# tatsy/normalizing-flows-pytorch

Hardware: AMD Instinct MI355X
Metric: samples/sec (train step: forward flow + log-det + NLL + backward + Adam) (higher is better)
Workload: dtype f32; 1 GPU; Glow CIFAR-shape (3,32,32) L=3 K=32 batch 64 per GPU (512 over 8); per_gpu_batch=64, global_batch=64, parallelism=dp1, hipgraph=True, deterministic=True, dp_one_graph=False

## Files before the change

include/nfhip.h:

```cpp
#ifndef NFHIP_H
#define NFHIP_H

#include <stdint.h>

#ifdef __cplusplus
extern "C" {
#endif

typedef void* nf_stream_t;

enum nf_split_mode {
    NF_SPLIT_1D = 0,
    NF_SPLIT_CHECKER = 1,
    NF_SPLIT_CHANNEL = 2,
    NF_SPLIT_NONE = 3
};

enum nf_chan_op {
    NF_ACTNORM = 0,
    NF_FLOWBN = 1
};

#define NF_E_BADARG 10001
#define NF_E_UNSUPPORTED 10002
// ... 332 lines not shown
    const float* cp_out;
    const float* cp_a;
    const float* cp_c;
    float* cp_g_z;
    float* cp_g_out;
    float* cp_g_a;
    float* cp_g_c;
    int cp_mode, cp_odd, cp_C;
    int ws_gen;
    float* g_gamma[5];
    float* g_beta[5];
    const float* wpk[6];
    const float* hd_g_h;
    const float* hd_W;
    const float* hd_ls;
} nf_convnet_bwd_desc;
int nf_convnet_chain_bwd(const nf_convnet_bwd_desc* desc, int64_t B, int I0, int O_out, int H, int W, int training,
                         nf_stream_t stream);
int nf_convnet_chain_bwd_run(const nf_convnet_bwd_desc* descs, int n, int64_t B, int I0, int O_out, int H, int W, int training,
                             nf_stream_t stream);

#define NF_CONV_PACK_IMAGE_FLOATS (3 * 36 * 128)
#define NF_CONV_PACK_MAX_LAYERS 1024
typedef struct nf_conv_pack_desc {
    const float* w;
    float* dst;
    int O, I, ksize, reserved;
} nf_conv_pack_desc;
int nf_conv_weight_pack_images(int O, int I, int ksize);
int nf_conv_weight_pack(const nf_conv_pack_desc* descs, int n, nf_stream_t stream);
// ... 450 lines not shown
```

normalizing-flows-pytorch_amd/csrc/conv_bn.hip:

```cpp
#include <mutex>
#include <unordered_set>
#include <vector>

#include "nf_common.h"
#include "nf_det.h"

NF_DET_STATE(nf_cvb)
NF_DET_HOST_API(nf_cvb)

#include "nf_conv_core.h"

#ifdef NF_CV_PROF
__device__ long long nf_cv_prof[32];
#define NF_CV_STAMP(i)                                                                 \
    do {                                                                               \
        if (blockIdx.x == 0 && threadIdx.x == 0) nf_cv_prof[i] = wall_clock64();       \
    } while (0)
extern "C" int nf_cv_prof_read(long long* out) {
    return (int)hipMemcpyFromSymbol(out, HIP_SYMBOL(nf_cv_prof), sizeof(long long) * 32);
}
#else
#define NF_CV_STAMP(i)
#endif

// ... 917 lines not shown
}
static_assert(sizeof(nf_conv_bwd_desc) % sizeof(unsigned) == 0, "descriptor: whole words");

static int nf_conv_bn_wgrad_launch(nf_conv_bwd_desc* descs, const nf_conv_bwd_desc* tab, int n, int slabs, int64_t B, int I, int O, int H,
                                   int W, int ksize, nf_stream_t stream) {
    NfCvGeo g;
    if (descs == nullptr || n < 1 || (tab == nullptr && n > NF_CV_WG_MAX) || n > NF_CONV_WGRAD_TABLE_MAX ||
        !nf_conv_bn_usable(B > 0 ? B : 1, I, O, H, W, ksize))
        return NF_E_BADARG;
    if (B == 0) return 0;
    if (!nf_cv_geometry(g, B, H, W, ksize)) return NF_E_BADARG;
    if (!nf_cv_fits_int32(B, I > O ? I : O, H * W)) return NF_E_BADARG;
    if (!nf_cv_set_valid(g, descs[0].valid_h, descs[0].valid_w)) return NF_E_BADARG;
    const bool masked = nf_cv_masked(g);
    bool one_plain = true;
    for (int k = 0; k < n; ++k) {
        if (descs[k].valid_h != descs[0].valid_h || descs[k].valid_w != descs[0].valid_w) return NF_E_BADARG;
        if (descs[k].g_weff == nullptr || descs[k].in == nullptr) return NF_E_BADARG;
        if (descs[k].bn_gamma != nullptr && I > 32) return NF_E_BADARG;
        if (descs[k].gn_src != nullptr && O > 32) return NF_E_BADARG;
        descs[k].g_store = nullptr; descs[k].gn_out = nullptr; descs[k].sum_g = nullptr; descs[k].sum_gx = nullptr;
        one_plain = one_plain && !(descs[k].g_direct != nullptr && descs[k].g_skip != nullptr);
    }
    NfCvBwdMulti m{};
    hipStream_t st = (hipStream_t)stream;
    if (tab == nullptr) {
        for (int k = 0; k < n; ++k) m.d[k] = descs[k];
    } else {
        for (int k0 = 0; k0 < n; k0 += NF_CV_DESC_WRITE) {
            const int cnt = n - k0 < NF_CV_DESC_WRITE ? n - k0 : NF_CV_DESC_WRITE;
            NfCvDescChunk w{};
            for (int k = 0; k < cnt; ++k) w.d[k] = descs[k0 + k];
            hipLaunchKernelGGL(k_conv_desc_write, dim3(1), dim3(256), 0, st, w, const_cast<nf_conv_bwd_desc*>(tab) + k0, cnt);
        }
        m = NfCvBwdMulti{};
    }
    const int ICB = (I + 31) / 32, OCB = (O + 31) / 32;
    const int T = ksize * ksize;
    const size_t lds = sizeof(float) * ((size_t)32 * g.CS + (size_t)32 * OCB * g.CS + 5 * 32 + 4 * 32 + 2 * 4 * 32);
    if (slabs < 1 || slabs > NF_CV_BWD_MAX_SLABS || slabs > g.tiles) return NF_E_BADARG;
    const unsigned grid = (unsigned)slabs;
    if (!masked && one_plain && nf_conv_bulk_wgrad_plan(B, I, O, H, W, ksize))
        return nf_conv_bulk_wgrad(tab == nullptr ? m.d : nullptr, tab, n, B, I, H, W, (int)grid, st);
    const int iters = (int)((g.tiles + grid - 1) / grid);
    int rc;
    const size_t lds_lean = sizeof(float) * ((size_t)2 * 64 * g.CS + 5 * 32 + 2 * 32);
    const bool lean = !masked && ICB == 1 && OCB == 1 && B * (int64_t)(I > O ? I : O) * H * W < ((int64_t)1 << 30) && 64 * g.CS >= T * 1024 &&
                      lds_lean <= 160 * 1024;
#define NF_LAUNCH(T_, IB_, OB_, LEAN_)                                                                                 \
    do {                                                                                                               \
        const size_t lds_ = LEAN_ ? lds_lean : lds;                                                                    \
        rc = nf_cv_optin(k_conv_bn_wgrad_multi<T_, IB_, OB_, LEAN_>, lds_);                                            \
        if (rc) return rc;                                                                                             \
        hipLaunchKernelGGL((k_conv_bn_wgrad_multi<T_, IB_, OB_, LEAN_>), dim3(grid, (unsigned)n), dim3(NF_CV_THREADS), lds_, st, m, \
                           tab, g, I, O, iters);                                                                       \
    } while (0)
    if (T == 9) {
        if (ICB == 1 && lean) NF_LAUNCH(9, 1, 1, true);
// ... 96 lines not shown
```

normalizing-flows-pytorch_amd/csrc/conv_bulk.hip:

```cpp
#include <cstdlib>
#include <mutex>
#include <type_traits>
#include <unordered_set>

#include "nf_common.h"
#include "nf_det.h"

NF_DET_STATE(nf_cbk)
NF_DET_HOST_API(nf_cbk)

#include "nf_conv_core.h"

#include "nf_bf16x3.h"

#ifdef NF_CB_PROF
__device__ long long nf_cb_prof[64];
#define NF_CB_STAMP(i)                                                                 \
    do {                                                                               \
        if (blockIdx.x == 0 && threadIdx.x == 0 && (i) < 64) nf_cb_prof[i] = wall_clock64(); \
    } while (0)
extern "C" int nf_cb_prof_read(long long* out) { return (int)hipMemcpyFromSymbol(out, HIP_SYMBOL(nf_cb_prof), sizeof(long long) * 64); }
#define NF_CBW_STAMP(T, i)                                                             \
    do {                                                                               \
        if (blockIdx.x == 0 && blockIdx.y == 0 && threadIdx.x == (T) && (i) >= 0 && (i) < 64) nf_cb_prof[i] = wall_clock64(); \
// ... 667 lines not shown
}
__device__ __forceinline__ const float* nf_cbw_pin(const float* p) {
    const uint64_t a = (uint64_t)p;
    const unsigned lo = __builtin_amdgcn_readfirstlane((unsigned)a), hi = __builtin_amdgcn_readfirstlane((unsigned)(a >> 32));
    return (const float*)(((uint64_t)hi << 32) | lo);
}
__device__ __forceinline__ void nf_cbw_put4(char* p, int plane_bytes, const float (&v)[4]) {
    bf16x2 h0, m0, l0, h1, m1, l1;
    nf_cc_split2(f32x2{v[0], v[1]}, h0, m0, l0);
    nf_cc_split2(f32x2{v[2], v[3]}, h1, m1, l1);
    *(bf16x4*)(p) = bf16x4{h0[0], h0[1], h1[0], h1[1]};
    *(bf16x4*)(p + plane_bytes) = bf16x4{m0[0], m0[1], m1[0], m1[1]};
    *(bf16x4*)(p + 2 * plane_bytes) = bf16x4{l0[0], l0[1], l1[0], l1[1]};
}

__global__ void __launch_bounds__(NF_CBW_THREADS) k_conv3_bulk_wgrad(NfCbwMulti m, const nf_conv_bwd_desc* __restrict__ tab, NfCbwGeo g, int I) {
    extern __shared__ __attribute__((aligned(16))) float smem[];
    const nf_conv_bwd_desc& d = tab != nullptr ? tab[blockIdx.y] : m.d[blockIdx.y];
    char* const lds = (char*)smem;
    const int PA = 32 * g.ACH, PG = 32 * NF_CBW_GCH;
    const int BUF = 3 * (PA + PG);
    float* cst = (float*)(lds + 2 * BUF);
    const int tid = threadIdx.x, lane = tid & 63, wid = __builtin_amdgcn_readfirstlane(tid >> 6), c32 = lane & 31, hs = lane >> 5;
    const bool walker = wid < 4;
    const bool has_bn = d.bn_gamma != nullptr, has_src = d.gn_src != nullptr;
    const int64_t Npx = g.B * g.HW;

    for (int e = tid; e < 2 * BUF / 16; e += NF_CBW_THREADS) *(u32x4*)(lds + 16 * e) = u32x4{0u, 0u, 0u, 0u};
    if (tid < 32) {
        const int oo = tid;
        float c1 = 0.f, mean = 0.f, invstd = 0.f, mg = 0.f, mgx = 0.f;
        if (has_src) {
            invstd = d.cbn_save_invstd[oo]; mean = d.cbn_save_mean[oo]; c1 = d.cbn_gamma[oo] * invstd;
            if (d.cbn_sum_g != nullptr) {
#pragma unroll
                for (int r = 0; r < NF_STAT_REPL; ++r) { mg += d.cbn_sum_g[32 * r + oo]; mgx += d.cbn_sum_gx[32 * r + oo]; }
                const float invN = 1.f / (float)Npx;
                mg *= invN; mgx *= invN;
            }
        }
// ... 135 lines not shown
                const bool ok = (cls == 1u || (cls == 2u && top) || (cls == 3u && bot)) && sm < brem;
                okm |= (ok ? 1u : 0u) << r;
                rx[S][r] = nf_cbw_ld128(rxs, ok ? xoff[r] : NF_CB_OOB);
            }
            xok[S] = okm;
            unsigned go[4], gp[4], gs[4];
#pragma unroll
            for (int r = 0; r < 4; ++r) {
                go[r] = pv ? goff0 + (unsigned)r * gcstep : NF_CB_OOB;
                gp[r] = plain != nullptr ? go[r] : NF_CB_OOB;
                gs[r] = has_src ? go[r] : NF_CB_OOB;
            }
            const __amdgpu_buffer_rsrc_t rr = nf_cb_rsrc(plain + gbase);
#pragma unroll
            for (int r = 0; r < 4; ++r) rp[S][r] = nf_cbw_ld128(rr, gp[r]);
            const __amdgpu_buffer_rsrc_t r3 = nf_cb_rsrc(p_src + gbase), r4 = nf_cb_rsrc(p_out + gbase);
#pragma unroll
            for (int r = 0; r < 4; ++r) { rs[S][r] = nf_cbw_ld128(r3, gs[r]); ro[S][r] = nf_cbw_ld128(r4, gs[r]); }
        };
        auto convert = [&](auto SET) {
            constexpr int S = decltype(SET)::value;
            char* fa = lds + S * BUF;
            char* fg = fa + 3 * PA;
#pragma unroll
            for (int r = 0; r < NF_CBW_MAXR; ++r)
                if (r < g.nr && ((xmeta >> (4 * r)) & 4u)) {
                    const bool ok = (xok[S] >> r) & 1u;
                    const float xsc = kx[r][0], xsh = kx[r][1];
                    float v[4];
#pragma unroll
                    for (int j = 0; j < 4; ++j) {
                        float x = rx[S][r][j];
                        if (has_bn) x = fmaxf(fmaf(x, xsc, xsh), 0.f);
                        v[j] = ok ? x : 0.f;
                    }
                    nf_cbw_put4(fa + xlds[r], PA, v);
                }
            float kg[4][5];
            if (has_src) {
#pragma unroll
                for (int r = 0; r < 4; ++r)
#pragma unroll
                    for (int q = 0; q < 5; ++q) kg[r][q] = cst[32 * q + 8 * r + gch0];
            }
#pragma unroll
            for (int r = 0; r < 4; ++r) {
                float v[4] = {0.f, 0.f, 0.f, 0.f};
                if (plain != nullptr) {
#pragma unroll
                    for (int j = 0; j < 4; ++j) v[j] = rp[S][r][j];
                }
                if (has_src) {
                    const float kc1 = kg[r][0], kmean = kg[r][1], kinv = kg[r][2], kmg = kg[r][3], kmgx = kg[r][4];
#pragma unroll
                    for (int j = 0; j < 4; ++j) {
                        const float xh = (ro[S][r][j] - kmean) * kinv;
                        v[j] += kc1 * (rs[S][r][j] - kmg - xh * kmgx);
                    }
                }
#pragma unroll
                for (int j = 0; j < 4; ++j) v[j] = gok[S] ? v[j] : 0.f;
                gsum[r] += (v[0] + v[1]) + (v[2] + v[3]);
                nf_cbw_put4(fg + glds0 + r * 8 * NF_CBW_GCH, PG, v);
            }
        };
        using S0 = std::integral_constant<int, 0>;
        using S1 = std::integral_constant<int, 1>;
        const int64_t n = tile0 < g.tiles ? (g.tiles - tile0 + tstep - 1) / tstep : 0;
        issue(S0{}, tile0);
        issue(S1{}, tile0 + tstep);
        if (n > 0) convert(S0{});
        issue(S0{}, tile0 + 2 * tstep);
// ... 394 lines not shown
#undef NF_CB_FWD2
#undef NF_CB_FWD3
    if (rc) return rc;
    NF_CHECK_LAUNCH();
    return 0;
}

extern "C" int nf_conv_bulk_wgrad_plan(int64_t B, int I, int O, int H, int W, int ksize) {
    const int on = 1;
    const int64_t min_px = nf_cb_min_px() == 16384 + 1 ? 4096 : nf_cb_min_px() - 1;
    if (!on || !nf_cb_on() || ksize != 3 || O != 32 || I < 1 || I > 32 || B * H * W < min_px) return 0;
    NfCbwGeo g;
    return nf_cbw_geometry(g, B, H, W) ? 1 : 0;
}
int nf_conv_bulk_wgrad(const nf_conv_bwd_desc* descs, const nf_conv_bwd_desc* tab, int n, int64_t B, int I, int H, int W, int slabs,
                       hipStream_t st) {
    NfCbwGeo g;
    if (!nf_cbw_geometry(g, B, H, W) || n < 1 || slabs < 1 || (descs == nullptr) == (tab == nullptr)) return NF_E_BADARG;
    if (descs != nullptr && n > NF_CONV_WGRAD_MAX) return NF_E_BADARG;
    NfCbwMulti m{};
    if (descs != nullptr)
        for (int k = 0; k < n; ++k) m.d[k] = descs[k];
    const size_t lds = nf_cbw_lds_bytes(g);
    int rc = nf_cb_optin(k_conv3_bulk_wgrad);
    if (rc) return rc;
    const unsigned gx = (unsigned)(g.tiles < slabs ? g.tiles : slabs);
    if ((int)gx != slabs) return NF_E_BADARG;
    hipLaunchKernelGGL(k_conv3_bulk_wgrad, dim3(gx, (unsigned)n), dim3(NF_CBW_THREADS), lds, st, m, tab, g, I);
    NF_CHECK_LAUNCH();
    return 0;
}

int nf_conv_bulk_bwd_plan(const nf_conv_bwd_desc* d, int64_t B, int I, int O, int H, int W, int ksize) {
    if (!nf_cb_on() || ksize != 3 || O != 32 || I < 1 || I > 32 || B * H * W < nf_cb_min_px()) return 0;
    if (d->g_weff != nullptr || d->g_bias != nullptr || d->g_direct != nullptr || d->gn_src == nullptr || d->out == nullptr) return 0;
    if (!(B * 32 * (int64_t)H * W < (int64_t)1 << 31)) return 0;
    NfCbGeo cg;
    return nf_cb_plan(cg, B, 32, H, W, 4, nf_cb_force_nblk());
}

int nf_conv_bulk_bwd(const nf_conv_bwd_desc* desc, int64_t B, int I, int H, int W, hipStream_t st) {
    NfCbGeo cg;
    const int nblk = nf_cb_plan(cg, B, 32, H, W, 4, nf_cb_force_nblk());
// ... 34 lines not shown
```

normalizing-flows-pytorch_amd/csrc/conv_chain.hip:

```cpp
#include <cstdlib>
#include <cstring>
#include <mutex>
#include <unordered_set>
#include "nf_conv_core.h"
#include "nf_det.h"

NF_DET_STATE(nf_ccd)
NF_DET_HOST_API(nf_ccd)
#include "nf_bf16x3.h"
#include "nf_small_plu.h"

#define NF_CC_NL 6
#define NF_CC_NB 5
#define NF_CC_MAX_BLOCKS NF_CONVNET_MAX_BLOCKS

#define NF_CC_WG_SLOTS (NF_CC_NB * NF_CC_MAX_BLOCKS * 64)
#define NF_CC_GROUP 16
#define NF_CC_MAX_GROUPS ((NF_CC_MAX_BLOCKS + NF_CC_GROUP - 1) / NF_CC_GROUP)
#define NF_CC_FLAT_MAX 128
#define NF_CC_STAT_SLOTS (NF_CC_WG_SLOTS + NF_CC_NB * NF_CC_MAX_GROUPS * 64)
static_assert(2 * NF_CC_STAT_SLOTS == NF_CONVNET_WS_FLOATS, "exchange workspace size in include/nfhip.h");

NF_PERSIST_STATE(nf_cc)
NF_PERSIST_HOST_API(nf_cc)
// ... 1544 lines not shown
        nrows = (G + NF_CC_GROUP - 1) / NF_CC_GROUP;
    }
    nf_cc_collect_slots<RUN>(xs, rs, gen, nrows, XS);
    peek();
    __syncthreads();
    {
        float pa = 0.f, pb = 0.f;
        for (int b = l; b < nrows; b += 32) { pa += xs[b * XS + ci]; pb += xs[b * XS + 32 + ci]; }
        const float A = nf_cc_sum32(pa), Bs = nf_cc_sum32(pb);
        if (l == 0) { tot[ci] = A; tot[32 + ci] = Bs; }
    }
    __syncthreads();
    return tot;
}

template <int NPB, int NKQ, bool HALO, bool CPL, int FWc, int CSc, bool PK, bool RUN>
__device__ __forceinline__ void nf_cc_bwd_step(const nf_convnet_bwd_desc& d, const NfCvGeo& g, int I0, int O_out, int training,
                                               const NfSplit& cs) {
    static_assert(NPB * NKQ == NF_CV_WAVES, "sixteen waves");
    constexpr int OWN = 16 / NKQ, PXW = 32 * NPB;
    extern __shared__ __attribute__((aligned(16))) float sm[];
    const NfCcLds L = nf_cc_lds<NPB, NKQ>(g.CS, 1);
    float* Wl = sm + L.WL;
    float* RS = sm + L.RS;
    float* kc = sm + L.KC;
    float* red = sm + L.RED;
    const int CSr = FWc > 0 ? CSc : g.CS;
    const int WPs = L.WPs;
    const int tid = nf_cc_step_tid<RUN>();
    const int lane = tid & 63, wid = tid >> 6, c32 = lane & 31, hs = lane >> 5;
// ... 205 lines not shown
                atomicAdd(d.cp_g_a, ta);
                atomicAdd(d.cp_g_c, tc);
            }
        }
        nf_cc_ksplit_exchange<NKQ>(own, acc, RS, pb, kq, lane);
        NF_CC_STAMP(67 + 6 * (4 - l));
        float* gn = d.gn[l];
#pragma unroll
        for (int rr = 0; rr < OWN; ++rr) {
            const int oc = nf_cv_cd_row(OWN * kq + rr, hs);
            const float a = xh[rr];
            const bool keep = pv && fmaf(a, kc[oc], kc[32 + oc]) > 0.f;
            const float v = keep ? own[rr] : 0.f;
            own[rr] = v;
            xh[rr] = (a - kc[64 + oc]) * kc[96 + oc];
            if (pv) gn[(b * 32 + oc) * g.HW + q] = v;
        }
        if (halo) nf_cc_halo_publish<OWN>(hslots, gbase, l, g, (int)tile, y0, px, kq, hs, own);
        float mg[OWN], mgx[OWN];
        unsigned long long hw[2] = {0ull, 0ull};
        const float* tot;
        {
            float p2[OWN], S1, S2;
            int which;
#pragma unroll
            for (int rr = 0; rr < OWN; ++rr) p2[rr] = own[rr] * xh[rr];
            nf_cc_half_sums2<OWN>(own, p2, c32, S1, S2, which);
            if (c32 < OWN) {
                const int oc = nf_cv_cd_row(OWN * kq + which, hs);
                red[pb * 32 + oc] = S1;
                red[NPB * 32 + pb * 32 + oc] = S2;
// ... 5 lines not shown
            if (stash) {
                if (blockIdx.x == 0 && nf_cc_tidx<RUN>() < 64) sm[ST + 64 * l + nf_cc_tidx<RUN>()] = tot[nf_cc_tidx<RUN>()];
            } else if (blockIdx.x == 0 && nf_cc_tidx<RUN>() < 64) {
                (nf_cc_tidx<RUN>() < 32 ? d.sum_g[l] : d.sum_gx[l])[nf_cc_tidx<RUN>() & 31] = tot[nf_cc_tidx<RUN>()];
                float* sink = nf_cc_tidx<RUN>() < 32 ? d.g_beta[l] : d.g_gamma[l];
                if (sink != nullptr) sink[nf_cc_tidx<RUN>() & 31] += tot[nf_cc_tidx<RUN>()];
            }
#pragma unroll
            for (int rr = 0; rr < OWN; ++rr) {
                const int oc = nf_cv_cd_row(OWN * kq + rr, hs);
                mg[rr] = training ? tot[oc] * invN : 0.f;
                mgx[rr] = training ? tot[32 + oc] * invN : 0.f;
            }
        }
        const bool on_stream = (l & 1) == 0;
        float* gs = (l == 4) ? d.g_store[0] : (l == 2 ? d.g_store[1] : nullptr);
#pragma unroll
        for (int rr = 0; rr < OWN; ++rr) {
            const int oc = nf_cv_cd_row(OWN * kq + rr, hs);
            float G = kc[oc] * (own[rr] - mg[rr] - xh[rr] * mgx[rr]);
            if (on_stream) G += gstream[rr];
            G = pv ? G : 0.f;
            own[rr] = G;
            if (on_stream) gstream[rr] = G;
            if (gs != nullptr && pv) gs[(b * 32 + oc) * g.HW + q] = G;
        }
#pragma unroll
        for (int j = 0; j < OWN / 4; ++j) {
            const int c0 = nf_cv_cd_row(OWN * kq + 4 * j, hs);
            nf_cc_frame_store4(Fr, CSr, c0, fpos, own[4 * j], own[4 * j + 1], own[4 * j + 2], own[4 * j + 3]);
        }
        if constexpr (OWN == 2) nf_cc_frame_store2(Fr, CSr, nf_cv_cd_row(OWN * kq, hs), fpos, own[0], own[1]);
        if constexpr (OWN == 1) nf_cc_frame_store1(Fr, CSr, nf_cv_cd_row(kq, hs), fpos, own[0]);
        if (halo && nf_cc_tidx<RUN>() < 32 * g.W) {
            const int c = nf_cc_tidx<RUN>() >> g.lgW;
            const float mgc = training ? tot[c] * invN : 0.f, mgxc = training ? tot[32 + c] * invN : 0.f;
#pragma unroll
            for (int s2 = 0; s2 < 2; ++s2) {
                float v = 0.f;
                const int f = nf_cc_halo_poll(hslots, gbase, l, g, (int)tile, y0, s2, v, hw[s2]);
// ... 390 lines not shown
    NF_CHECK_LAUNCH();
    return 0;
}

static int nf_cc_bwd_args(const nf_convnet_bwd_desc* desc, int64_t B, int I0, int O_out, int H, int W, NfSplit& cs, NfCvGeo& g, int& PX) {
    if (desc == nullptr || !nf_convnet_chain_usable(B, I0, O_out, H, W)) return NF_E_BADARG;
    memset(&cs, 0, sizeof(cs));
    if (desc->cp_g_y != nullptr) {
        if (desc->cp_g_ld == nullptr || desc->cp_z == nullptr || desc->cp_out == nullptr || desc->cp_a == nullptr || desc->cp_c == nullptr ||
            desc->cp_g_z == nullptr || desc->cp_g_out == nullptr || desc->cp_g_a == nullptr || desc->cp_g_c == nullptr)
            return NF_E_BADARG;
        if (!nf_cc_coupling_split(cs, desc->cp_mode, desc->cp_odd, desc->cp_C, I0, O_out, H, W)) return NF_E_BADARG;
    } else if (desc->g_out == nullptr) {
        return NF_E_BADARG;
    }
    PX = nf_cc_tile_px(B, H, W);
    if (!nf_cv_geometry(g, B, H, W, 3, PX)) return NF_E_BADARG;
    if (desc->hd_g_h != nullptr) {
        const bool small = desc->cp_C >= 2 && desc->cp_C <= 4;
        if (desc->cp_g_y == nullptr || desc->hd_W == nullptr || desc->hd_ls == nullptr || (!small && (desc->cp_C < 9 || desc->cp_C > 64)) ||
            ((cs.H * cs.W) & 15) != 0 || (H * W > PX && cs.W < 16) || (int64_t)(O_out >> 1) * PX > NF_CC_HD_X1_MAX)
            return NF_E_BADARG;
    }
    const bool pk = desc->wpk[0] != nullptr;
    for (int i = 1; i < NF_CC_NL; ++i)
        if ((desc->wpk[i] != nullptr) != pk) return NF_E_BADARG;
    return 0;
}

extern "C" int nf_convnet_chain_bwd(const nf_convnet_bwd_desc* desc, int64_t B, int I0, int O_out, int H, int W, int training,
// ... 122 lines not shown
```

normalizing-flows-pytorch_amd/csrc/nf_conv_core.h:

```cpp
#pragma once
#include "nf_common.h"

typedef float f32x16 __attribute__((ext_vector_type(16)));

#define NF_CV_WAVES 16
#define NF_CV_THREADS (NF_CV_WAVES * NF_WAVE)
#define NF_CV_PX 128
#define NF_CV_MAX_FRAME 384
#define NF_CV_FJ (NF_CV_MAX_FRAME / NF_WAVE)
#define NF_CV_CU (32 / NF_CV_WAVES)
#define NF_CV_MAX_I 96
#define NF_CV_MAX_O 192
#define NF_CV_WS 33
#define NF_CV_RS (NF_CV_WAVES * 12 * NF_WAVE)

struct NfCvGeo {
    int H, W, HW;
    int TH;
    int SEG;
    int halo;
    int FW, FS;
    int FSZ;
    int CS;
    int lgW, lgSP;
// ... 271 lines not shown
            sc = d.bn_gamma[k] * invstd;
            sh = d.bn_beta[k] - mean * sc;
        }
        kc[k] = sc;
        kc[32 + k] = sh;
    }
    if (training && d.bn_gamma != nullptr && d.bn_num_batches != nullptr && blockIdx.x == 0 && threadIdx.x == 0)
        d.bn_num_batches[0] += 1;
}

int nf_conv_bulk_fwd_plan(const nf_conv_desc* d, int64_t B, int I, int O, int H, int W, int ksize);
int nf_conv_bulk_fwd(const nf_conv_desc* desc, int64_t B, int I, int H, int W, int training, float eps, float mom, hipStream_t st);
int nf_conv_bulk_bwd_plan(const nf_conv_bwd_desc* d, int64_t B, int I, int O, int H, int W, int ksize);
int nf_conv_bulk_bwd(const nf_conv_bwd_desc* desc, int64_t B, int I, int H, int W, hipStream_t st);
extern "C" int nf_conv_bulk_wgrad_plan(int64_t B, int I, int O, int H, int W, int ksize);
int nf_conv_bulk_wgrad(const nf_conv_bwd_desc* descs, const nf_conv_bwd_desc* tab, int n, int64_t B, int I, int H, int W, int slabs, hipStream_t st);
int nf_conv1_bulk_fwd_plan(const nf_conv_desc* d, int64_t B, int I, int O, int H, int W, int ksize);
int nf_conv1_bulk_fwd(const nf_conv_desc* desc, int64_t B, int O, int H, int W, int training, float eps, float mom, hipStream_t st);
int nf_conv1_bulk_bwd_plan(const nf_conv_bwd_desc* d, int64_t B, int I, int O, int H, int W, int ksize);
int nf_conv1_bulk_bwd(const nf_conv_bwd_desc* desc, int64_t B, int O, int H, int W, hipStream_t st);
```

normalizing-flows-pytorch_amd/fused_conv.py:

```python
import ctypes
import functools

import torch

from . import _native as N
from . import workspace as WS
from .fused import BN_EPS, BN_MOMENTUM, H, R, _desc

WS_ROWS = 2 * R + 2
GB = 256

_FWD_FIELDS = ['in_', 'weight', 'bias', 'residual', 'out', 'bn_gamma', 'bn_beta', 'bn_sum', 'bn_sqsum', 'bn_center',
               'bn_running_mean', 'bn_running_var', 'bn_num_batches', 'bn_save_mean', 'bn_save_invstd', 'stat_sum',
               'stat_sqsum', 'wpk']
_BWD_FIELDS = ['in_', 'weight', 'bn_gamma', 'bn_beta', 'bn_save_mean', 'bn_save_invstd', 'g_direct', 'g_skip', 'gn_src',
               'out', 'cbn_gamma', 'cbn_save_mean', 'cbn_save_invstd', 'cbn_sum_g', 'cbn_sum_gx', 'g_store', 'g_bias',
               'g_weff', 'gn_out', 'sum_g', 'sum_gx', 'wpk']


class ConvDesc(ctypes.Structure):
    _fields_ = [(f, ctypes.c_void_p) for f in _FWD_FIELDS] + [('valid_h', ctypes.c_int), ('valid_w', ctypes.c_int)]


class ConvBwdDesc(ctypes.Structure):
# ... 18 lines not shown
                ('hs_P', ctypes.c_void_p), ('hs_L', ctypes.c_void_p), ('hs_U', ctypes.c_void_p), ('hs_Lm', ctypes.c_void_p),
                ('hs_Um', ctypes.c_void_p), ('hs_sign', ctypes.c_void_p), ('hs_Wout', ctypes.c_void_p),
                ('ws_gen', ctypes.c_int), ('ws_reserved', ctypes.c_int)]


class ConvNetBwdDesc(ctypes.Structure):
    _fields_ = [('w', ctypes.c_void_p * 6), ('gamma', ctypes.c_void_p * 5), ('beta', ctypes.c_void_p * 5),
                ('save_mean', ctypes.c_void_p * 5), ('save_invstd', ctypes.c_void_p * 5), ('acts', ctypes.c_void_p * 5),
                ('g_out', ctypes.c_void_p), ('gn', ctypes.c_void_p * 5), ('sum_g', ctypes.c_void_p * 5),
                ('sum_gx', ctypes.c_void_p * 5), ('g_store', ctypes.c_void_p * 2), ('g_x', ctypes.c_void_p),
                ('ws_zero', ctypes.c_void_p),
                ('cp_g_y', ctypes.c_void_p), ('cp_g_ld', ctypes.c_void_p), ('cp_z', ctypes.c_void_p), ('cp_out', ctypes.c_void_p),
                ('cp_a', ctypes.c_void_p), ('cp_c', ctypes.c_void_p), ('cp_g_z', ctypes.c_void_p), ('cp_g_out', ctypes.c_void_p),
                ('cp_g_a', ctypes.c_void_p), ('cp_g_c', ctypes.c_void_p), ('cp_mode', ctypes.c_int), ('cp_odd', ctypes.c_int),
                ('cp_C', ctypes.c_int), ('ws_gen', ctypes.c_int), ('g_gamma', ctypes.c_void_p * 5), ('g_beta', ctypes.c_void_p * 5),
                ('wpk', ctypes.c_void_p * 6), ('hd_g_h', ctypes.c_void_p), ('hd_W', ctypes.c_void_p), ('hd_ls', ctypes.c_void_p)]


class ConvPackDesc(ctypes.Structure):
    _fields_ = [('w', ctypes.c_void_p), ('dst', ctypes.c_void_p), ('O', ctypes.c_int), ('I', ctypes.c_int), ('ksize', ctypes.c_int),
                ('reserved', ctypes.c_int)]


CONV_PACK_ON = True


def pack_conv_weights(wn_modules, w_effs):
    if not CONV_PACK_ON:
        return
    lib = N.load()
    img = N.header_constant('NF_CONV_PACK_IMAGE_FLOATS')
# ... 187 lines not shown
            launch_small_head_params(heads)
        if plu:
            from .fused import PluDesc, _plu_launch
            from .fused import _desc as _fdesc
            _plu_launch('nf_invconv_weight_bwd_multi',
                        [_fdesc(PluDesc, g_W=gW, P=P, L=L, U=U, L_mask=Lm, U_mask=Um, sign_s=sg, log_s=ls, g_ld=sgld, g_L=gL, g_U=gU,
                                g_log_s=gls, B=1, C=C, accumulate=1, pixels=float(px))
                         for gW, P, L, U, Lm, Um, sg, ls, sgld, gL, gU, gls, C, px in plu])
        if not layers and not sums:
            return
        self.launch_layers(layers)
        _slab_sum_all(sums)


WGRAD_FROM_STORE = True
WGRAD_TABLE = True
CONV_DEFER_ON = True
CONV_DEFER = ConvDefer()


CHAIN_SLOTS_SHARED = True


def _chain_slots(n, dev):
    A = WS.ARENA
    if not (CHAIN_SLOTS_SHARED and A.active and A.buf is not None and A.buf.device == dev):
        return WS.zeros(n, dev), 0
    t = A.step_state.get('chain_slots')
    if t is None or t.numel() < n:
        t = A.step_state['chain_slots'] = WS.zeros(n, dev)
# ... 325 lines not shown
    B, Hh, Ww = shape
    valid = getattr(ctx, 'valid', None)
    vk = dict(valid_h=valid[0], valid_w=valid[1]) if valid else {}
    if valid:
        gs = g_out.new_zeros(B, O_out, Hh, Ww)
        gs[:, :, :valid[0], :valid[1]] = g_out
        g_out = gs
    g_out = g_out.contiguous() if cpl is None else torch.empty_like(cpl[1])
    slabs = int(N.load().nf_conv_bwd_slabs(B, Hh, Ww))
    chained = CONV_CHAIN_BWD_ON and not valid and _chain_usable(B, I0, O_out, Hh, Ww)
    g_weff = [None] * nl if ((ctx.defer and CONV_DEFER.active) or chained) else \
        [torch.empty(slabs, t.numel(), dtype=torch.float32, device=dev) for t in w]
    acc = WS.zeros(nl * R * GB + nb * 2 * R * H, dev)
    g_bias = [acc[i * R * GB:(i + 1) * R * GB] for i in range(nl)]
    sums = acc[nl * R * GB:].view(nb, 2, R * H)
    gn = [torch.empty_like(acts[0]) for _ in range(nb)]
    g_x = torch.empty_like(x) if (cpl is None and ctx.needs_input_grad[0]) else None
    G_skip = None

    def in_bn(j):
        return dict(bn_gamma=gamma[j], bn_beta=beta[j], bn_save_mean=ws[j, 2 * R], bn_save_invstd=ws[j, 2 * R + 1])

    def cons_bn(j):
        return dict(cbn_gamma=gamma[j], cbn_save_mean=ws[j, 2 * R], cbn_save_invstd=ws[j, 2 * R + 1],
                    cbn_sum_g=sums[j, 0] if training else None, cbn_sum_gx=sums[j, 1] if training else None)

    defer = ctx.defer and CONV_DEFER.active
    if cpl is not None and not chained:
        raise RuntimeError('the fused coupling needs the chain kernels in both directions')
    queued = []
    stores = [torch.empty_like(acts[0]) for _ in range(2)] if chained else None

    def layer(I, O, k, i, **kw):
        kw.update(vk)
        if not defer and not chained:
            _bwd(shape, I, O, k, g_bias=g_bias[i], g_weff=g_weff[i], **kw)
            return
        if not chained:
            _bwd(shape, I, O, k, **kw)
        wkw = {f: v for f, v in kw.items() if f not in ('g_store', 'gn_out', 'sum_g', 'sum_gx')}
        if WGRAD_FROM_STORE and kw.get('g_store') is not None:
            wkw = {f: v for f, v in wkw.items() if f not in ('gn_src', 'out', 'g_skip') and not f.startswith('cbn_')}
            wkw['g_direct'] = kw['g_store']
        wkw['g_bias'] = g_bias[i]
        queued.append(((shape, I, O, k, valid), wkw, i))

    if chained:
        d = ConvNetBwdDesc()
        for i in range(nl):
            d.w[i] = w[i].data_ptr()
        for j in range(nb):
            d.gamma[j], d.beta[j] = gamma[j].data_ptr(), beta[j].data_ptr()
            d.save_mean[j], d.save_invstd[j] = ws[j, 2 * R].data_ptr(), ws[j, 2 * R + 1].data_ptr()
            d.acts[j], d.gn[j] = acts[j].data_ptr(), gn[j].data_ptr()
            d.sum_g[j], d.sum_gx[j] = sums[j, 0].data_ptr(), sums[j, 1].data_ptr()
        d.g_out = g_out.data_ptr()
        d.g_store[0], d.g_store[1] = stores[0].data_ptr(), stores[1].data_ptr()
        d.g_x = g_x.data_ptr() if g_x is not None else None
        if getattr(ctx, 'packs', None) is not None and all(p.current() for p in ctx.packs):
            for i in range(nl):
                d.wpk[i] = ctx.packs[i].data_ptr()
        slots, d.ws_gen = _chain_slots(_chain_ws_floats(B, I0, O_out, Hh, Ww), dev)
        d.ws_zero = slots.data_ptr()
        if ctx.sinks is not None:
            for j in range(nb):
                d.g_gamma[j], d.g_beta[j] = ctx.sinks[nl + 2 * j].data_ptr(), ctx.sinks[nl + 2 * j + 1].data_ptr()
        pend, g_z = None, None
        if cpl is not None:
            z, out, a, c = cpl
            g_y, g_ld = cpl_grads
            g_z = torch.empty_like(z)
            if ctx.cpl_sinks is not None:
# ... 7 lines not shown
            d.cp_a, d.cp_c, d.cp_g_z, d.cp_g_out, d.cp_g_a, d.cp_g_c = a.data_ptr(), c.data_ptr(), g_z.data_ptr(), g_out.data_ptr(), pa, pc
            d.cp_mode, d.cp_odd = ctx.cpl_meta
            d.cp_C = z.shape[1]
            from . import functional as NF
            pend = NF.PENDING_HEAD_BWD.pop(g_y.data_ptr(), None)
            if pend is not None:
                hg, hls, hW, hgx, small = pend
                Cz = z.shape[1]
                fits = (9 <= Cz <= 64) if small is None else (2 <= Cz <= 4)
                if hgx.shape == z.shape and hg.shape == z.shape and hg.is_contiguous() and fits:
                    d.hd_g_h, d.hd_W, d.hd_ls = hg.data_ptr(), hW.data_ptr(), hls.data_ptr()
                else:
                    NF.flush_pending_head_bwd(pend)
        collect = bool(defer) and cpl is not None and ctx.cpl_sinks is not None
        RUNS.launch_bwd(ctx, d, (B, I0, O_out, Hh, Ww, int(training), bool(d.wpk[0])),
                        (saved, cpl_grads, g_out, gn, stores, acc, slots, g_z, g_x, pend, getattr(ctx, 'packs', None)), collect, bool(d.hd_g_h))

    layer(H, O_out, 1, nl - 1, in_=acts[nb - 1], weight=w[nl - 1], g_direct=g_out, gn_out=gn[nb - 1], sum_g=sums[nb - 1, 0],
          sum_gx=sums[nb - 1, 1], **in_bn(nb - 1))
    cpk = getattr(ctx, 'packs', None)
    pk = (lambda i: cpk[i].buf) if (cpk is not None and all(p.current() for p in cpk)) else (lambda i: None)
    for j in range(nb - 1, 0, -1):
        is_stream = (j % 2 == 0)
        store = (stores[(nb - 1 - j) // 2] if chained else torch.empty_like(acts[0])) if is_stream else None
        layer(H, H, 3, j, in_=acts[j - 1], weight=w[j], gn_src=gn[j], out=acts[j], g_skip=G_skip if is_stream else None,
              g_store=store, gn_out=gn[j - 1], sum_g=sums[j - 1, 0], sum_gx=sums[j - 1, 1], wpk=pk(j), **in_bn(j - 1), **cons_bn(j))
        if is_stream:
            G_skip = store
    layer(I0, H, 3, 0, in_=x, weight=w[0], gn_src=gn[0], out=acts[0], g_skip=G_skip, gn_out=g_x, wpk=pk(0), **cons_bn(0))

    direct = ctx.sinks is not None
    g_w = [torch.empty_like(t) for t in w]
    if direct:
        d_bias = ctx.sinks[:nl]
        d_bn = [tuple(ctx.sinks[nl + 2 * j:nl + 2 * j + 2]) for j in range(nb)]
    else:
        d_bias = [torch.empty(t.shape[0], dtype=torch.float32, device=dev) for t in w]
        d_bn = [(torch.empty(H, dtype=torch.float32, device=dev), torch.empty(H, dtype=torch.float32, device=dev))
                for _ in range(nb)]
    jobs = [(g_weff[i], g_w[i], w[i].numel(), w[i].numel(), slabs, False, w[i].shape[2] * w[i].shape[3]) for i in range(nl)]
    jobs += [(g_bias[i], d_bias[i], w[i].shape[0], GB, R, direct, 1) for i in range(nl)]
    bn_jobs = []
    if not (chained and direct):
        for j in range(nb):
# ... 82 lines not shown
```

Baseline: 2894 samples/s.

## Store final gradients for every chain layer so wgrad skips BN-backward recompute

The chained conv-net backward kernel now writes the fully combined pre-activation gradient G for every layer into new store slots (g_store_more), not only for the two stream layers. The raw gn buffers are dropped. The weight-gradient pass reads these stored gradients directly. The bulk wgrad kernel is templated on HAS_SRC, so when no layer needs the BN-backward reconstruction it skips the extra src/out loads and arithmetic. This trades extra stores in the chain kernel for fewer loads and less recompute in the wgrad kernel.

```diff
diff --git a/include/nfhip.h b/include/nfhip.h
--- a/include/nfhip.h
+++ b/include/nfhip.h
@@ -370,6 +370,7 @@
     const float* hd_g_h;
     const float* hd_W;
     const float* hd_ls;
+    float* g_store_more[3];
 } nf_convnet_bwd_desc;
 int nf_convnet_chain_bwd(const nf_convnet_bwd_desc* desc, int64_t B, int I0, int O_out, int H, int W, int training,
                          nf_stream_t stream);
diff --git a/normalizing-flows-pytorch_amd/csrc/conv_bn.hip b/normalizing-flows-pytorch_amd/csrc/conv_bn.hip
--- a/normalizing-flows-pytorch_amd/csrc/conv_bn.hip
+++ b/normalizing-flows-pytorch_amd/csrc/conv_bn.hip
@@ -955,6 +955,7 @@
     if (!nf_cv_set_valid(g, descs[0].valid_h, descs[0].valid_w)) return NF_E_BADARG;
     const bool masked = nf_cv_masked(g);
     bool one_plain = true;
+    bool any_src = false;
     for (int k = 0; k < n; ++k) {
         if (descs[k].valid_h != descs[0].valid_h || descs[k].valid_w != descs[0].valid_w) return NF_E_BADARG;
         if (descs[k].g_weff == nullptr || descs[k].in == nullptr) return NF_E_BADARG;
@@ -962,6 +963,7 @@
         if (descs[k].gn_src != nullptr && O > 32) return NF_E_BADARG;
         descs[k].g_store = nullptr; descs[k].gn_out = nullptr; descs[k].sum_g = nullptr; descs[k].sum_gx = nullptr;
         one_plain = one_plain && !(descs[k].g_direct != nullptr && descs[k].g_skip != nullptr);
+        any_src = any_src || descs[k].gn_src != nullptr;
     }
     NfCvBwdMulti m{};
     hipStream_t st = (hipStream_t)stream;
@@ -982,7 +984,7 @@
     if (slabs < 1 || slabs > NF_CV_BWD_MAX_SLABS || slabs > g.tiles) return NF_E_BADARG;
     const unsigned grid = (unsigned)slabs;
     if (!masked && one_plain && nf_conv_bulk_wgrad_plan(B, I, O, H, W, ksize))
-        return nf_conv_bulk_wgrad(tab == nullptr ? m.d : nullptr, tab, n, B, I, H, W, (int)grid, st);
+        return nf_conv_bulk_wgrad(tab == nullptr ? m.d : nullptr, tab, n, B, I, H, W, (int)grid, any_src, st);
     const int iters = (int)((g.tiles + grid - 1) / grid);
     int rc;
     const size_t lds_lean = sizeof(float) * ((size_t)2 * 64 * g.CS + 5 * 32 + 2 * 32);
diff --git a/normalizing-flows-pytorch_amd/csrc/conv_bulk.hip b/normalizing-flows-pytorch_amd/csrc/conv_bulk.hip
--- a/normalizing-flows-pytorch_amd/csrc/conv_bulk.hip
+++ b/normalizing-flows-pytorch_amd/csrc/conv_bulk.hip
@@ -705,6 +705,7 @@
     *(bf16x4*)(p + 2 * plane_bytes) = bf16x4{l0[0], l0[1], l1[0], l1[1]};
 }
 
+template <bool HAS_SRC>
 __global__ void __launch_bounds__(NF_CBW_THREADS) k_conv3_bulk_wgrad(NfCbwMulti m, const nf_conv_bwd_desc* __restrict__ tab, NfCbwGeo g, int I) {
     extern __shared__ __attribute__((aligned(16))) float smem[];
     const nf_conv_bwd_desc& d = tab != nullptr ? tab[blockIdx.y] : m.d[blockIdx.y];
@@ -714,7 +715,7 @@
     float* cst = (float*)(lds + 2 * BUF);
     const int tid = threadIdx.x, lane = tid & 63, wid = __builtin_amdgcn_readfirstlane(tid >> 6), c32 = lane & 31, hs = lane >> 5;
     const bool walker = wid < 4;
-    const bool has_bn = d.bn_gamma != nullptr, has_src = d.gn_src != nullptr;
+    const bool has_bn = d.bn_gamma != nullptr, has_src = HAS_SRC && d.gn_src != nullptr;
     const int64_t Npx = g.B * g.HW;
 
     for (int e = tid; e < 2 * BUF / 16; e += NF_CBW_THREADS) *(u32x4*)(lds + 16 * e) = u32x4{0u, 0u, 0u, 0u};
@@ -880,9 +881,11 @@
             const __amdgpu_buffer_rsrc_t rr = nf_cb_rsrc(plain + gbase);
 #pragma unroll
             for (int r = 0; r < 4; ++r) rp[S][r] = nf_cbw_ld128(rr, gp[r]);
-            const __amdgpu_buffer_rsrc_t r3 = nf_cb_rsrc(p_src + gbase), r4 = nf_cb_rsrc(p_out + gbase);
-#pragma unroll
-            for (int r = 0; r < 4; ++r) { rs[S][r] = nf_cbw_ld128(r3, gs[r]); ro[S][r] = nf_cbw_ld128(r4, gs[r]); }
+            if constexpr (HAS_SRC) {
+                const __amdgpu_buffer_rsrc_t r3 = nf_cb_rsrc(p_src + gbase), r4 = nf_cb_rsrc(p_out + gbase);
+#pragma unroll
+                for (int r = 0; r < 4; ++r) { rs[S][r] = nf_cbw_ld128(r3, gs[r]); ro[S][r] = nf_cbw_ld128(r4, gs[r]); }
+            }
         };
         auto convert = [&](auto SET) {
             constexpr int S = decltype(SET)::value;
@@ -903,11 +906,13 @@
                     nf_cbw_put4(fa + xlds[r], PA, v);
                 }
             float kg[4][5];
-            if (has_src) {
-#pragma unroll
-                for (int r = 0; r < 4; ++r)
-#pragma unroll
-                    for (int q = 0; q < 5; ++q) kg[r][q] = cst[32 * q + 8 * r + gch0];
+            if constexpr (HAS_SRC) {
+                if (has_src) {
+#pragma unroll
+                    for (int r = 0; r < 4; ++r)
+#pragma unroll
+                        for (int q = 0; q < 5; ++q) kg[r][q] = cst[32 * q + 8 * r + gch0];
+                }
             }
 #pragma unroll
             for (int r = 0; r < 4; ++r) {
@@ -916,12 +921,14 @@
 #pragma unroll
                     for (int j = 0; j < 4; ++j) v[j] = rp[S][r][j];
                 }
-                if (has_src) {
-                    const float kc1 = kg[r][0], kmean = kg[r][1], kinv = kg[r][2], kmg = kg[r][3], kmgx = kg[r][4];
-#pragma unroll
-                    for (int j = 0; j < 4; ++j) {
-                        const float xh = (ro[S][r][j] - kmean) * kinv;
-                        v[j] += kc1 * (rs[S][r][j] - kmg - xh * kmgx);
+                if constexpr (HAS_SRC) {
+                    if (has_src) {
+                        const float kc1 = kg[r][0], kmean = kg[r][1], kinv = kg[r][2], kmg = kg[r][3], kmgx = kg[r][4];
+#pragma unroll
+                        for (int j = 0; j < 4; ++j) {
+                            const float xh = (ro[S][r][j] - kmean) * kinv;
+                            v[j] += kc1 * (rs[S][r][j] - kmg - xh * kmgx);
+                        }
                     }
                 }
 #pragma unroll
@@ -1346,7 +1353,7 @@
     return nf_cbw_geometry(g, B, H, W) ? 1 : 0;
 }
 int nf_conv_bulk_wgrad(const nf_conv_bwd_desc* descs, const nf_conv_bwd_desc* tab, int n, int64_t B, int I, int H, int W, int slabs,
-                       hipStream_t st) {
+                       bool any_src, hipStream_t st) {
     NfCbwGeo g;
     if (!nf_cbw_geometry(g, B, H, W) || n < 1 || slabs < 1 || (descs == nullptr) == (tab == nullptr)) return NF_E_BADARG;
     if (descs != nullptr && n > NF_CONV_WGRAD_MAX) return NF_E_BADARG;
@@ -1354,11 +1361,12 @@
     if (descs != nullptr)
         for (int k = 0; k < n; ++k) m.d[k] = descs[k];
     const size_t lds = nf_cbw_lds_bytes(g);
-    int rc = nf_cb_optin(k_conv3_bulk_wgrad);
+    int rc = any_src ? nf_cb_optin(k_conv3_bulk_wgrad<true>) : nf_cb_optin(k_conv3_bulk_wgrad<false>);
     if (rc) return rc;
     const unsigned gx = (unsigned)(g.tiles < slabs ? g.tiles : slabs);
     if ((int)gx != slabs) return NF_E_BADARG;
-    hipLaunchKernelGGL(k_conv3_bulk_wgrad, dim3(gx, (unsigned)n), dim3(NF_CBW_THREADS), lds, st, m, tab, g, I);
+    if (any_src) hipLaunchKernelGGL(k_conv3_bulk_wgrad<true>, dim3(gx, (unsigned)n), dim3(NF_CBW_THREADS), lds, st, m, tab, g, I);
+    else hipLaunchKernelGGL(k_conv3_bulk_wgrad<false>, dim3(gx, (unsigned)n), dim3(NF_CBW_THREADS), lds, st, m, tab, g, I);
     NF_CHECK_LAUNCH();
     return 0;
 }
diff --git a/normalizing-flows-pytorch_amd/csrc/conv_chain.hip b/normalizing-flows-pytorch_amd/csrc/conv_chain.hip
--- a/normalizing-flows-pytorch_amd/csrc/conv_chain.hip
+++ b/normalizing-flows-pytorch_amd/csrc/conv_chain.hip
@@ -1582,6 +1582,10 @@
     return tot;
 }
 
+__host__ __device__ __forceinline__ float* nf_cc_grad_slot(const nf_convnet_bwd_desc& d, int l) {
+    return (l & 1) ? d.g_store_more[(3 - l) >> 1] : (l == 0 ? d.g_store_more[2] : d.g_store[(4 - l) >> 1]);
+}
+
 template <int NPB, int NKQ, bool HALO, bool CPL, int FWc, int CSc, bool PK, bool RUN>
 __device__ __forceinline__ void nf_cc_bwd_step(const nf_convnet_bwd_desc& d, const NfCvGeo& g, int I0, int O_out, int training,
                                                const NfSplit& cs) {
@@ -1817,7 +1821,7 @@
             const float v = keep ? own[rr] : 0.f;
             own[rr] = v;
             xh[rr] = (a - kc[64 + oc]) * kc[96 + oc];
-            if (pv) gn[(b * 32 + oc) * g.HW + q] = v;
+            if (pv && gn != nullptr) gn[(b * 32 + oc) * g.HW + q] = v;
         }
         if (halo) nf_cc_halo_publish<OWN>(hslots, gbase, l, g, (int)tile, y0, px, kq, hs, own);
         float mg[OWN], mgx[OWN];
@@ -1853,16 +1857,21 @@
             }
         }
         const bool on_stream = (l & 1) == 0;
-        float* gs = (l == 4) ? d.g_store[0] : (l == 2 ? d.g_store[1] : nullptr);
+        float* gs = nf_cc_grad_slot(d, l);
 #pragma unroll
         for (int rr = 0; rr < OWN; ++rr) {
             const int oc = nf_cv_cd_row(OWN * kq + rr, hs);
-            float G = kc[oc] * (own[rr] - mg[rr] - xh[rr] * mgx[rr]);
-            if (on_stream) G += gstream[rr];
+            const float t = own[rr] - mg[rr] - xh[rr] * mgx[rr];
+            float G = kc[oc] * t;
+            float Gw = G;
+            if (on_stream) {
+                Gw = l == 0 ? fmaf(kc[oc], t, gstream[rr]) : G + gstream[rr];
+                G += gstream[rr];
+            }
             G = pv ? G : 0.f;
             own[rr] = G;
             if (on_stream) gstream[rr] = G;
-            if (gs != nullptr && pv) gs[(b * 32 + oc) * g.HW + q] = G;
+            if (gs != nullptr && pv) gs[(b * 32 + oc) * g.HW + q] = Gw;
         }
 #pragma unroll
         for (int j = 0; j < OWN / 4; ++j) {
@@ -2283,6 +2292,8 @@
     } else if (desc->g_out == nullptr) {
         return NF_E_BADARG;
     }
+    for (int l = 0; l < NF_CC_NB; ++l)
+        if (desc->gn[l] == nullptr && nf_cc_grad_slot(*desc, l) == nullptr) return NF_E_BADARG;
     PX = nf_cc_tile_px(B, H, W);
     if (!nf_cv_geometry(g, B, H, W, 3, PX)) return NF_E_BADARG;
     if (desc->hd_g_h != nullptr) {
diff --git a/normalizing-flows-pytorch_amd/csrc/nf_conv_core.h b/normalizing-flows-pytorch_amd/csrc/nf_conv_core.h
--- a/normalizing-flows-pytorch_amd/csrc/nf_conv_core.h
+++ b/normalizing-flows-pytorch_amd/csrc/nf_conv_core.h
@@ -309,7 +309,8 @@
 int nf_conv_bulk_bwd_plan(const nf_conv_bwd_desc* d, int64_t B, int I, int O, int H, int W, int ksize);
 int nf_conv_bulk_bwd(const nf_conv_bwd_desc* desc, int64_t B, int I, int H, int W, hipStream_t st);
 extern "C" int nf_conv_bulk_wgrad_plan(int64_t B, int I, int O, int H, int W, int ksize);
-int nf_conv_bulk_wgrad(const nf_conv_bwd_desc* descs, const nf_conv_bwd_desc* tab, int n, int64_t B, int I, int H, int W, int slabs, hipStream_t st);
+int nf_conv_bulk_wgrad(const nf_conv_bwd_desc* descs, const nf_conv_bwd_desc* tab, int n, int64_t B, int I, int H, int W, int slabs, bool any_src,
+                       hipStream_t st);
 int nf_conv1_bulk_fwd_plan(const nf_conv_desc* d, int64_t B, int I, int O, int H, int W, int ksize);
 int nf_conv1_bulk_fwd(const nf_conv_desc* desc, int64_t B, int O, int H, int W, int training, float eps, float mom, hipStream_t st);
 int nf_conv1_bulk_bwd_plan(const nf_conv_bwd_desc* d, int64_t B, int I, int O, int H, int W, int ksize);
diff --git a/normalizing-flows-pytorch_amd/fused_conv.py b/normalizing-flows-pytorch_amd/fused_conv.py
--- a/normalizing-flows-pytorch_amd/fused_conv.py
+++ b/normalizing-flows-pytorch_amd/fused_conv.py
@@ -56,7 +56,8 @@
                 ('cp_a', ctypes.c_void_p), ('cp_c', ctypes.c_void_p), ('cp_g_z', ctypes.c_void_p), ('cp_g_out', ctypes.c_void_p),
                 ('cp_g_a', ctypes.c_void_p), ('cp_g_c', ctypes.c_void_p), ('cp_mode', ctypes.c_int), ('cp_odd', ctypes.c_int),
                 ('cp_C', ctypes.c_int), ('ws_gen', ctypes.c_int), ('g_gamma', ctypes.c_void_p * 5), ('g_beta', ctypes.c_void_p * 5),
-                ('wpk', ctypes.c_void_p * 6), ('hd_g_h', ctypes.c_void_p), ('hd_W', ctypes.c_void_p), ('hd_ls', ctypes.c_void_p)]
+                ('wpk', ctypes.c_void_p * 6), ('hd_g_h', ctypes.c_void_p), ('hd_W', ctypes.c_void_p), ('hd_ls', ctypes.c_void_p),
+                ('g_store_more', ctypes.c_void_p * 3)]
 
 
 class ConvPackDesc(ctypes.Structure):
@@ -274,6 +275,7 @@
 
 
 WGRAD_FROM_STORE = True
+WGRAD_STORE_ALL = True
 WGRAD_TABLE = True
 CONV_DEFER_ON = True
 CONV_DEFER = ConvDefer()
@@ -629,7 +631,9 @@
     acc = WS.zeros(nl * R * GB + nb * 2 * R * H, dev)
     g_bias = [acc[i * R * GB:(i + 1) * R * GB] for i in range(nl)]
     sums = acc[nl * R * GB:].view(nb, 2, R * H)
-    gn = [torch.empty_like(acts[0]) for _ in range(nb)]
+    store_all = WGRAD_FROM_STORE and WGRAD_STORE_ALL
+    G_all = [torch.empty_like(acts[0]) for _ in range(nb)] if (chained and store_all) else None
+    gn = [torch.empty_like(acts[0]) for _ in range(nb)] if G_all is None else [None] * nb
     g_x = torch.empty_like(x) if (cpl is None and ctx.needs_input_grad[0]) else None
     G_skip = None
 
@@ -644,7 +648,7 @@
     if cpl is not None and not chained:
         raise RuntimeError('the fused coupling needs the chain kernels in both directions')
     queued = []
-    stores = [torch.empty_like(acts[0]) for _ in range(2)] if chained else None
+    stores = ([G_all[4], G_all[2]] if G_all is not None else [torch.empty_like(acts[0]) for _ in range(2)]) if chained else None
 
     def layer(I, O, k, i, **kw):
         kw.update(vk)
@@ -667,10 +671,13 @@
         for j in range(nb):
             d.gamma[j], d.beta[j] = gamma[j].data_ptr(), beta[j].data_ptr()
             d.save_mean[j], d.save_invstd[j] = ws[j, 2 * R].data_ptr(), ws[j, 2 * R + 1].data_ptr()
-            d.acts[j], d.gn[j] = acts[j].data_ptr(), gn[j].data_ptr()
+            d.acts[j], d.gn[j] = acts[j].data_ptr(), (gn[j].data_ptr() if gn[j] is not None else None)
             d.sum_g[j], d.sum_gx[j] = sums[j, 0].data_ptr(), sums[j, 1].data_ptr()
         d.g_out = g_out.data_ptr()
         d.g_store[0], d.g_store[1] = stores[0].data_ptr(), stores[1].data_ptr()
+        if G_all is not None:
+            for k, j in enumerate((3, 1, 0)):
+                d.g_store_more[k] = G_all[j].data_ptr()
         d.g_x = g_x.data_ptr() if g_x is not None else None
         if getattr(ctx, 'packs', None) is not None and all(p.current() for p in ctx.packs):
             for i in range(nl):
@@ -708,7 +715,7 @@
                     NF.flush_pending_head_bwd(pend)
         collect = bool(defer) and cpl is not None and ctx.cpl_sinks is not None
         RUNS.launch_bwd(ctx, d, (B, I0, O_out, Hh, Ww, int(training), bool(d.wpk[0])),
-                        (saved, cpl_grads, g_out, gn, stores, acc, slots, g_z, g_x, pend, getattr(ctx, 'packs', None)), collect, bool(d.hd_g_h))
+                        (saved, cpl_grads, g_out, gn, stores, G_all, acc, slots, g_z, g_x, pend, getattr(ctx, 'packs', None)), collect, bool(d.hd_g_h))
 
     layer(H, O_out, 1, nl - 1, in_=acts[nb - 1], weight=w[nl - 1], g_direct=g_out, gn_out=gn[nb - 1], sum_g=sums[nb - 1, 0],
           sum_gx=sums[nb - 1, 1], **in_bn(nb - 1))
@@ -716,12 +723,18 @@
     pk = (lambda i: cpk[i].buf) if (cpk is not None and all(p.current() for p in cpk)) else (lambda i: None)
     for j in range(nb - 1, 0, -1):
         is_stream = (j % 2 == 0)
-        store = (stores[(nb - 1 - j) // 2] if chained else torch.empty_like(acts[0])) if is_stream else None
+        if G_all is not None:
+            store = G_all[j]
+        elif is_stream:
+            store = stores[(nb - 1 - j) // 2] if chained else torch.empty_like(acts[0])
+        else:
+            store = torch.empty_like(acts[0]) if (store_all and defer and not chained) else None
         layer(H, H, 3, j, in_=acts[j - 1], weight=w[j], gn_src=gn[j], out=acts[j], g_skip=G_skip if is_stream else None,
               g_store=store, gn_out=gn[j - 1], sum_g=sums[j - 1, 0], sum_gx=sums[j - 1, 1], wpk=pk(j), **in_bn(j - 1), **cons_bn(j))
         if is_stream:
             G_skip = store
-    layer(I0, H, 3, 0, in_=x, weight=w[0], gn_src=gn[0], out=acts[0], g_skip=G_skip, gn_out=g_x, wpk=pk(0), **cons_bn(0))
+    layer(I0, H, 3, 0, in_=x, weight=w[0], gn_src=gn[0], out=acts[0], g_skip=G_skip, gn_out=g_x, wpk=pk(0),
+          g_store=G_all[0] if G_all is not None else None, **cons_bn(0))
 
     direct = ctx.sinks is not None
     g_w = [torch.empty_like(t) for t in w]
```

Result: no change. 2867 samples/s (-0.9%).
